# wyf0912/ContextGS

Hardware: AMD Instinct MI355X
Metric: views/sec fwd+bwd @1920×1080, 1M anchors (higher is better)
Workload: dtype f32

## Files before the change

contextgs_amd/csrc/mlp3.hip:

```cpp
#include "cgs_internal.h"
#include "mlp_frag.h"
#include "buf_access.h"

#define M3_IN 54
#define M3_HID 50
#define M3_NTI 4
#define M3_XP 64
#define M3_NT1 4
#define M3_HP 64
#define M3_HCAT 150
#define M3_HLD 150
#define M3_HPITCH 50
#define M3_GLD 192
#define M3_GPITCH 64
#define M3_XLD 54
#ifndef M3_FWD_RT
#define M3_FWD_RT 1
#define M3_FWD_WAVES 16
#ifndef M3_FWD_LDS_STORE
#define M3_FWD_LDS_STORE 1
#endif
#ifndef M3W_ROUTER
#define M3W_ROUTER 1
#endif
#ifndef M3_TAILMAP
#define M3_TAILMAP 1
#endif
#define M3_FWD_PATCH (16 * 70)
#endif
#ifndef M3_BWD_RT
#define M3_BWD_RT 2
#define M3_BWD_WAVES 8
#endif

#ifndef M3_FUSED_WGRAD
#define M3_FUSED_WGRAD 1
#endif
#ifndef M3_PIPE
#define M3_PIPE 0
#endif
#define M3_FENCE()                         \
    do {                                   \
        asm volatile("" ::: "memory");     \
        __builtin_amdgcn_sched_barrier(0); \
    } while (0)

struct M3Head {
    const float *W1, *b1, *W2, *b2;
    float *Y;
    const float *dY;
    float *dZ2;
};

template <int OUT>
struct M3FwdLds {
    static constexpr int NT2 = (OUT + 15) / 16, OP = NT2 * 16;
    static constexpr int S1 = frag_pad4mod8(M3_HP), S2 = frag_pad4mod8(OP);
    static constexpr int FLOATS = M3_XP * S1 + M3_HP * S2 + M3_HP + OP;
};

template <int OUT>
__device__ __forceinline__ void m3_stage_fwd(float *lds, const M3Head &h, int tid, int nthr) {
    using L = M3FwdLds<OUT>;
    float *W1s = lds, *W2s = W1s + M3_XP * L::S1, *b1s = W2s + M3_HP * L::S2, *b2s = b1s + M3_HP;
    frag_stage_transposed<M3_IN, M3_HID, M3_XP, L::S1>(W1s, h.W1, tid, nthr);
    frag_stage_transposed<M3_HID, OUT, M3_HP, L::S2>(W2s, h.W2, tid, nthr);
    for (int i = tid; i < M3_HP; i += nthr) b1s[i] = i < M3_HID ? h.b1[i] : 0.f;
    for (int i = tid; i < L::OP; i += nthr) b2s[i] = i < OUT ? h.b2[i] : 0.f;
}

#define M3_MAX_ROWS (4ll << 20)
struct M3FwdBufs { ClBuf H, Y[3], Xo, X, src, feat, anc; };

template <int OUT, int ACT, int RT, bool TILED, bool TM>
__device__ __forceinline__ void m3_head_fwd(const float *lds, const M3Head &h, int head, const f32x4 (&xb)[RT][M3_NTI],
                                            const bool (&valid)[RT], int64_t row0, int g, int c,
                                            float *__restrict__ Hcat, const M3FwdBufs &B, float *patch) {
    using L = M3FwdLds<OUT>;
    const float *W1s = lds, *W2s = W1s + M3_XP * L::S1, *b1s = W2s + M3_HP * L::S2, *b2s = b1s + M3_HP;
    f32x4 acc1[M3_NT1][RT];
#pragma unroll
    for (int t = 0; t < M3_NT1; ++t)
#pragma unroll
        for (int rt = 0; rt < RT; ++rt) acc1[t][rt] = (f32x4){0.f, 0.f, 0.f, 0.f};
#if M3_PIPE
    float a1[2][4][M3_NT1];
#pragma unroll
    for (int j = 0; j < 4; ++j)
#pragma unroll
        for (int t = 0; t < M3_NT1; ++t) a1[0][j][t] = W1s[(4 * g + j) * L::S1 + 16 * t + c];
    auto krow = [&](int q, int j) { return (TM && q == M3_NTI - 1) ? 16 * q + g + 4 * j : 16 * q + 4 * g + j; };
#pragma unroll
    for (int q = 0; q < M3_NTI; ++q) {
        if (q + 1 < M3_NTI) {
#pragma unroll
            for (int j = 0; j < 4; ++j)
#pragma unroll
                for (int t = 0; t < M3_NT1; ++t)
                    a1[(q + 1) & 1][j][t] = W1s[krow(q + 1, j) * L::S1 + 16 * t + c];
        }
        M3_FENCE();
#pragma unroll
        for (int j = 0; j < 4; ++j) {
            if (16 * q + j >= M3_IN) continue;
            if (TM && q == M3_NTI - 1 && 16 * q + 4 * j >= M3_IN) continue;
#pragma unroll
            for (int t = 0; t < M3_NT1; ++t)
#pragma unroll
                for (int rt = 0; rt < RT; ++rt) acc1[t][rt] = frag_mfma(a1[q & 1][j][t], xb[rt][q][j], acc1[t][rt]);
        }
        M3_FENCE();
    }
#else
#pragma unroll
    for (int q = 0; q < M3_NTI; ++q)
#pragma unroll
        for (int j = 0; j < 4; ++j) {
            if (16 * q + j >= M3_IN) continue;
            if (TM && q == M3_NTI - 1 && 16 * q + 4 * j >= M3_IN) continue;
#pragma unroll
            for (int t = 0; t < M3_NT1; ++t) {
                const float a = W1s[((TM && q == M3_NTI - 1) ? 16 * q + g + 4 * j : 16 * q + 4 * g + j) * L::S1 + 16 * t + c];
#pragma unroll
                for (int rt = 0; rt < RT; ++rt) acc1[t][rt] = frag_mfma(a, xb[rt][q][j], acc1[t][rt]);
            }
        }
#endif
#pragma unroll
    for (int t = 0; t < M3_NT1; ++t)
#pragma unroll
        for (int rt = 0; rt < RT; ++rt) {
            const int64_t row = row0 + rt * 16 + c;
#pragma unroll
            for (int r = 0; r < 4; ++r) acc1[t][rt][r] = fmaxf(acc1[t][rt][r] + b1s[16 * t + 4 * g + r], 0.f);
            if (TILED)
                frag_tstore4<M3_HID>(B.H, (uint32_t)((row0 + rt * 16) >> 4) * (16 * M3_HLD * 4) + (uint32_t)head * (16 * M3_HID * 4), t, g, c,
                                     valid[rt], acc1[t][rt]);
            else
                frag_bstore4<M3_HID>(B.H, (uint32_t)row * (M3_HLD * 4) + (uint32_t)(M3_HPITCH * head) * 4, t, g, valid[rt], acc1[t][rt]);
        }
    f32x4 acc2[L::NT2][RT];
#pragma unroll
    for (int u = 0; u < L::NT2; ++u)
#pragma unroll
        for (int rt = 0; rt < RT; ++rt) acc2[u][rt] = (f32x4){0.f, 0.f, 0.f, 0.f};
#if M3_PIPE
    float a2[2][4][L::NT2];
#pragma unroll
    for (int r = 0; r < 4; ++r)
#pragma unroll
        for (int u = 0; u < L::NT2; ++u) a2[0][r][u] = W2s[(4 * g + r) * L::S2 + 16 * u + c];
#pragma unroll
    for (int t = 0; t < M3_NT1; ++t) {
        if (t + 1 < M3_NT1) {
#pragma unroll
            for (int r = 0; r < 4; ++r) {
                if (16 * (t + 1) + r >= M3_HID) continue;
#pragma unroll
                for (int u = 0; u < L::NT2; ++u) a2[(t + 1) & 1][r][u] = W2s[(16 * (t + 1) + 4 * g + r) * L::S2 + 16 * u + c];
            }
        }
        M3_FENCE();
#pragma unroll
        for (int r = 0; r < 4; ++r) {
            if (16 * t + r >= M3_HID) continue;
#pragma unroll
            for (int u = 0; u < L::NT2; ++u)
#pragma unroll
                for (int rt = 0; rt < RT; ++rt) acc2[u][rt] = frag_mfma(a2[t & 1][r][u], acc1[t][rt][r], acc2[u][rt]);
        }
        M3_FENCE();
    }
#else
#pragma unroll
    for (int t = 0; t < M3_NT1; ++t)
#pragma unroll
        for (int r = 0; r < 4; ++r) {
            if (16 * t + r >= M3_HID) continue;
#pragma unroll
            for (int u = 0; u < L::NT2; ++u) {
                const float a = W2s[(16 * t + 4 * g + r) * L::S2 + 16 * u + c];
#pragma unroll
                for (int rt = 0; rt < RT; ++rt) acc2[u][rt] = frag_mfma(a, acc1[t][rt][r], acc2[u][rt]);
            }
        }
#endif
#if M3_FWD_LDS_STORE
#pragma unroll
    for (int rt = 0; rt < RT; ++rt) {
        f32x4 yv[L::NT2];
#pragma unroll
        for (int u = 0; u < L::NT2; ++u)
#pragma unroll
            for (int r = 0; r < 4; ++r) yv[u][r] = frag_act<ACT>(acc2[u][rt][r] + b2s[16 * u + 4 * g + r]);
        frag_tile_store<OUT, L::NT2>(patch, B.Y[head], (uint32_t)(row0 + rt * 16) * (OUT * 4), yv, g, c, 16 * g + c);
    }
#else
#pragma unroll
    for (int u = 0; u < L::NT2; ++u)
#pragma unroll
        for (int rt = 0; rt < RT; ++rt) {
            const int64_t row = row0 + rt * 16 + c;
            f32x4 y;
#pragma unroll
            for (int r = 0; r < 4; ++r) y[r] = frag_act<ACT>(acc2[u][rt][r] + b2s[16 * u + 4 * g + r]);
            frag_bstore4<OUT>(B.Y[head], (uint32_t)row * (OUT * 4), u, g, valid[rt], y);
        }
#endif
}

struct M3Rows {
    const float *feat_src;
    const int64_t *src_row;
    const float *anchor;
    const float *cam;
    float *X_out;
    float *d_feat_src;
    float *d_anchor;
};

template <bool TM = false>
__device__ __forceinline__ f32x4 m3_load_x_rows_b(const M3FwdBufs &B, float cam0, float cam1, float cam2, int64_t row, int64_t srow,
                                                  int q, int g, bool valid) {
    const uint32_t fo = (uint32_t)srow * (M3_HID * 4);
    if (q < 3) return cl_l128(B.feat, cl_sel(valid, fo + (uint32_t)(16 * q + 4 * g) * 4));
    if (TM) {
        const f32x4 f2 = cl_l64(B.feat, cl_sel(valid && g < 2, fo + 48 * 4));
        const f32x4 a = cl_l96(B.anc, cl_sel(valid, (uint32_t)row * 12));
        const float ux = a[0] - cam0, uy = a[1] - cam1, uz = a[2] - cam2;
        const float dist = sqrtf(ux * ux + uy * uy + uz * uz);
        const float s0 = g == 0 ? f2[0] : (g == 1 ? f2[1] : (g == 2 ? ux / dist : uy / dist));
        const float s1 = g == 0 ? uz / dist : (g == 1 ? dist : 0.f);
        return valid ? (f32x4){s0, s1, 0.f, 0.f} : (f32x4){0.f, 0.f, 0.f, 0.f};
    }
    const f32x4 f2 = cl_l64(B.feat, cl_sel(valid && g == 0, fo + 48 * 4));
    const f32x4 a = cl_l96(B.anc, cl_sel(valid && g < 2, (uint32_t)row * 12));
    const float ux = a[0] - cam0, uy = a[1] - cam1, uz = a[2] - cam2;
    const float dist = sqrtf(ux * ux + uy * uy + uz * uz);
    const f32x4 v0 = (f32x4){f2[0], f2[1], ux / dist, uy / dist}, v1 = (f32x4){uz / dist, dist, 0.f, 0.f};
    const f32x4 z = (f32x4){0.f, 0.f, 0.f, 0.f};
    return !valid ? z : (g == 0 ? v0 : (g == 1 ? v1 : z));
}

template <int O0, int A0, int O1, int A1, int O2, int A2, int RT, int WAVES, bool ROWS, bool TILED = false>
__global__ void __launch_bounds__(WAVES * 64)
    mlp3_fwd_kernel(const float *__restrict__ X, int64_t ldx, M3Head h0, M3Head h1, M3Head h2,
                    float *__restrict__ Hcat, int64_t n, M3Rows R) {
    constexpr int WFL = M3FwdLds<O0>::FLOATS + M3FwdLds<O1>::FLOATS + M3FwdLds<O2>::FLOATS;
    static_assert(WFL % 4 == 0 && O0 <= 70 && O1 <= 70 && O2 <= 70 && M3_IN <= 70, "patch: 16-byte aligned, the widest image fits");
    __shared__ __attribute__((aligned(16))) float lds[WFL + (M3_FWD_LDS_STORE ? WAVES * M3_FWD_PATCH : 0)];
    float *l0 = lds, *l1 = l0 + M3FwdLds<O0>::FLOATS, *l2 = l1 + M3FwdLds<O1>::FLOATS;
    const int tid = threadIdx.x, nthr = WAVES * 64;
    float *patch = lds + WFL + (M3_FWD_LDS_STORE ? (tid >> 6) * M3_FWD_PATCH : 0);
    m3_stage_fwd<O0>(l0, h0, tid, nthr);
    m3_stage_fwd<O1>(l1, h1, tid, nthr);
    m3_stage_fwd<O2>(l2, h2, tid, nthr);
    __syncthreads();
    const int lane = tid & 63, wave = tid >> 6, g = lane >> 4, c = lane & 15;
    const int64_t ntiles = (n + 16 * RT - 1) / (16 * RT);
    f32x4 xb[RT][M3_NTI], xn[RT][M3_NTI];
    bool valid[RT], validn[RT];
    const int64_t tile0 = (int64_t)blockIdx.x * WAVES + wave, tstride = (int64_t)gridDim.x * WAVES;
    M3FwdBufs B;
    {
        const uint64_t nb = (uint64_t)n;
        const uint64_t nbt = (nb + 15) / 16 * 16;
        B.H = cl_buf(Hcat, (TILED ? nbt : nb) * (M3_HLD * 4));
        B.Y[0] = cl_buf(h0.Y, nb * (O0 * 4)); B.Y[1] = cl_buf(h1.Y, nb * (O1 * 4)); B.Y[2] = cl_buf(h2.Y, nb * (O2 * 4));
        B.Xo = cl_buf(ROWS ? R.X_out : nullptr, nb * (M3_XLD * 4));
        B.X = cl_buf(ROWS ? nullptr : X, nb > 0 ? ((nb - 1) * (uint64_t)ldx + M3_IN) * 4 : 0);
        B.src = cl_buf(ROWS ? R.src_row : nullptr, nb * 8);
        B.feat = cl_buf(ROWS ? R.feat_src : nullptr, CL_MAX_BYTES);
        B.anc = cl_buf(ROWS ? R.anchor : nullptr, nb * 12);
    }
    const float cam0 = ROWS ? R.cam[0] : 0.f, cam1 = ROWS ? R.cam[1] : 0.f, cam2 = ROWS ? R.cam[2] : 0.f;
    const uint32_t ldx4 = (uint32_t)ldx * 4;
    int64_t srow_n[RT], srow_nn[RT];
#pragma unroll
    for (int rt = 0; rt < RT; ++rt) {
        const int64_t row = tile0 * 16 * RT + rt * 16 + c, rown = row + tstride * 16 * RT;
        valid[rt] = tile0 < ntiles && row < n;
        const int64_t srow = ROWS ? cl_li64(B.src, cl_sel(valid[rt], (uint32_t)row * 8)) : 0;
        srow_n[rt] = ROWS ? cl_li64(B.src, cl_sel(rown < n, (uint32_t)rown * 8)) : 0;
#pragma unroll
        for (int q = 0; q < M3_NTI; ++q)
            xb[rt][q] = ROWS ? m3_load_x_rows_b<M3_TAILMAP>(B, cam0, cam1, cam2, row, srow, q, g, valid[rt])
                             : frag_bmask4<M3_IN>(frag_bload4<M3_IN>(B.X, (uint32_t)row * ldx4, q, g, valid[rt]), q, g);
    }
    for (int64_t tile = tile0; tile < ntiles; tile += tstride) {
        const int64_t row0 = tile * 16 * RT;
        asm volatile("" ::: "memory");
#pragma unroll
        for (int rt = 0; rt < RT; ++rt) {
            const int64_t row = (tile + tstride) * 16 * RT + rt * 16 + c, rownn = row + tstride * 16 * RT;
            validn[rt] = row < n;
            srow_nn[rt] = ROWS ? cl_li64(B.src, cl_sel(rownn < n, (uint32_t)rownn * 8)) : 0;
#pragma unroll
            for (int q = 0; q < M3_NTI; ++q)
                xn[rt][q] = ROWS ? m3_load_x_rows_b<M3_TAILMAP>(B, cam0, cam1, cam2, row, srow_n[rt], q, g, validn[rt])
                                 : frag_bmask4<M3_IN>(frag_bload4<M3_IN>(B.X, (uint32_t)row * ldx4, q, g, validn[rt]), q, g);
        }
        if (ROWS) {
#pragma unroll
            for (int rt = 0; rt < RT; ++rt)
#if M3_FWD_LDS_STORE
                if (R.X_out) {
                    if (M3_TAILMAP) {
#pragma unroll
                        for (int q = 0; q < M3_NTI - 1; ++q) cl_patch_put4(patch + c * M3_IN + 16 * q + 4 * g, xb[rt][q], 4);
                        patch[c * M3_IN + 48 + g] = xb[rt][M3_NTI - 1][0];
                        if (g < 2) patch[c * M3_IN + 52 + g] = xb[rt][M3_NTI - 1][1];
                        cl_patch_flush<64 * M3_IN>(patch, B.Xo, (uint32_t)(row0 + rt * 16) * (M3_XLD * 4), lane);
                    } else {
                        frag_tile_store<M3_IN, M3_NTI>(patch, B.Xo, (uint32_t)(row0 + rt * 16) * (M3_XLD * 4), xb[rt], g, c, lane);
                    }
                }
#else
#pragma unroll
                for (int q = 0; q < M3_NTI; ++q)
                    frag_bstore4<M3_IN>(B.Xo, (uint32_t)(row0 + rt * 16 + c) * (M3_XLD * 4), q, g, valid[rt], xb[rt][q]);
#endif
        }
        m3_head_fwd<O0, A0, RT, TILED, ROWS && M3_TAILMAP>(l0, h0, 0, xb, valid, row0, g, c, Hcat, B, patch);
        m3_head_fwd<O1, A1, RT, TILED, ROWS && M3_TAILMAP>(l1, h1, 1, xb, valid, row0, g, c, Hcat, B, patch);
        m3_head_fwd<O2, A2, RT, TILED, ROWS && M3_TAILMAP>(l2, h2, 2, xb, valid, row0, g, c, Hcat, B, patch);
#pragma unroll
        for (int rt = 0; rt < RT; ++rt) {
            valid[rt] = validn[rt];
            srow_n[rt] = srow_nn[rt];
#pragma unroll
            for (int q = 0; q < M3_NTI; ++q) xb[rt][q] = xn[rt][q];
        }
    }
}

template <int OUT>
struct M3BwdLds {
    static constexpr int NT2 = (OUT + 15) / 16, OP = NT2 * 16;
    static constexpr int SA = frag_pad4mod8(M3_HP), SB = frag_pad4mod8(M3_XP);
    static constexpr int FLOATS = OP * SA + M3_HP * SB;
};

template <int OUT>
__device__ __forceinline__ void m3_stage_bwd(float *lds, const M3Head &h, int tid, int nthr) {
    using L = M3BwdLds<OUT>;
    float *W2n = lds, *W1n = W2n + L::OP * L::SA;
    frag_stage_loop(h.W2, L::OP * L::SA, tid, nthr,
                    [](int i) { const int o = i / L::SA, hh = i % L::SA; return (o < OUT && hh < M3_HID) ? o * M3_HID + hh : -1; },
                    [&](int i, float v) { W2n[i] = v; });
    frag_stage_loop(h.W1, M3_HP * L::SB, tid, nthr,
                    [](int i) { const int hh = i / L::SB, k = i % L::SB; return (hh < M3_HID && k < M3_IN) ? hh * M3_IN + k : -1; },
                    [&](int i, float v) { W1n[i] = v; });
}

template <int OUT, int ACT, int RT>
__device__ __forceinline__ void m3_head_bwd(const float *lds, const M3Head &h, int head, const bool (&valid)[RT],
                                            int64_t row0, int g, int c, const float *__restrict__ Hcat,
                                            float *__restrict__ dZ1cat, f32x4 (&adx)[M3_NTI][RT]) {
    using L = M3BwdLds<OUT>;
    const float *W2n = lds, *W1n = W2n + L::OP * L::SA;
    f32x4 adh[M3_NT1][RT];
#pragma unroll
    for (int t = 0; t < M3_NT1; ++t)
#pragma unroll
        for (int rt = 0; rt < RT; ++rt) adh[t][rt] = (f32x4){0.f, 0.f, 0.f, 0.f};
    f32x4 b[L::NT2][RT], yv[L::NT2][RT], hv[M3_NT1][RT];
#pragma unroll
    for (int u = 0; u < L::NT2; ++u)
#pragma unroll
        for (int rt = 0; rt < RT; ++rt) {
            const int64_t row = row0 + rt * 16 + c;
            b[u][rt] = frag_load4<OUT>(h.dY + row * OUT, u, g, valid[rt]);
            if (ACT != FRAG_ACT_NONE) yv[u][rt] = frag_load4<OUT>(h.Y + row * OUT, u, g, valid[rt]);
        }
#pragma unroll
    for (int t = 0; t < M3_NT1; ++t)
#pragma unroll
        for (int rt = 0; rt < RT; ++rt)
            hv[t][rt] = frag_load4<M3_HID>(Hcat + (row0 + rt * 16 + c) * M3_HLD + M3_HPITCH * head, t, g, valid[rt]);
    if (ACT != FRAG_ACT_NONE) {
#pragma unroll
        for (int u = 0; u < L::NT2; ++u)
#pragma unroll
            for (int rt = 0; rt < RT; ++rt) {
#pragma unroll
                for (int r = 0; r < 4; ++r) b[u][rt][r] *= frag_act_grad<ACT>(yv[u][rt][r]);
                frag_store4<OUT>(h.dZ2 + (row0 + rt * 16 + c) * OUT, u, g, valid[rt], b[u][rt]);
            }
    }
#pragma unroll
    for (int u = 0; u < L::NT2; ++u)
#pragma unroll
        for (int j = 0; j < 4; ++j) {
            if (16 * u + j >= OUT) continue;
#pragma unroll
            for (int t = 0; t < M3_NT1; ++t) {
                const float a = W2n[(16 * u + 4 * g + j) * L::SA + 16 * t + c];
#pragma unroll
                for (int rt = 0; rt < RT; ++rt) adh[t][rt] = frag_mfma(a, b[u][rt][j], adh[t][rt]);
            }
        }
#pragma unroll
    for (int t = 0; t < M3_NT1; ++t)
#pragma unroll
        for (int rt = 0; rt < RT; ++rt) {
            const int64_t at = (row0 + rt * 16 + c) * M3_GLD + M3_GPITCH * head;
#pragma unroll
            for (int r = 0; r < 4; ++r) adh[t][rt][r] = hv[t][rt][r] > 0.f ? adh[t][rt][r] : 0.f;
// ... 55 lines not shown
                    dst[49] = adx[3][rt][1];
                    const float dvx = adx[3][rt][2], dvy = adx[3][rt][3], dvz = z52, dd = z53;
                    const float ux = R.anchor[3 * row] - R.cam[0], uy = R.anchor[3 * row + 1] - R.cam[1],
                                uz = R.anchor[3 * row + 2] - R.cam[2];
                    const float dist = sqrtf(ux * ux + uy * uy + uz * uz), inv = 1.f / dist;
                    const float vx = ux * inv, vy = uy * inv, vz = uz * inv;
                    const float dot = vx * dvx + vy * dvy + vz * dvz;
                    R.d_anchor[3 * row] = (dvx - vx * dot) * inv + vx * dd;
                    R.d_anchor[3 * row + 1] = (dvy - vy * dot) * inv + vy * dd;
                    R.d_anchor[3 * row + 2] = (dvz - vz * dot) * inv + vz * dd;
                }
            }
        } else if (dX) {
#pragma unroll
            for (int v = 0; v < M3_NTI; ++v)
#pragma unroll
                for (int rt = 0; rt < RT; ++rt)
                    frag_store4<M3_IN>(dX + (row0 + rt * 16 + c) * lddx, v, g, valid[rt], adx[v][rt]);
        }
    }
}


#define M3W_LD 20
#ifndef M3W_XPREFETCH
#define M3W_XPREFETCH 1
#endif
#define M3W_PATCH (16 * M3W_LD)
#ifndef M3W_PREFETCH_AT
#define M3W_PREFETCH_AT 2
#endif
#ifndef M3W_EARLY
#define M3W_EARLY 0
#endif
#define M3W_NPATCH 13
#define M3W_WAVES 4
#define M3W_E (M3_GLD * (M3_IN + 1) + (10 + 30 + 70) * (M3_HID + 1))

__device__ __forceinline__ f32x4 m3w_f2n(float *patch, f32x4 v, int g, int c) {
    *(f32x4 *)(patch + c * M3W_LD + 4 * g) = v;
    f32x4 o;
#pragma unroll
    for (int r = 0; r < 4; ++r) o[r] = patch[(4 * g + r) * M3W_LD + c];
    return o;
}

struct M3wBufs { ClBuf dY[3], Y[3], H, X; };
template <int OUT, int ACT>
struct M3wOps {
    static constexpr int NT2 = (OUT + 15) / 16;
    f32x4 dy[NT2], y[ACT != FRAG_ACT_NONE ? NT2 : 1], h[M3_NT1];
    template <bool TILED = false>
    __device__ __forceinline__ void load(const M3wBufs &B, int head, int64_t row, int g, bool valid) {
        const uint32_t ro = (uint32_t)row * (OUT * 4), rh = (uint32_t)row * (M3_HLD * 4) + (uint32_t)(M3_HPITCH * head) * 4;
        const uint32_t th = (uint32_t)(row >> 4) * (16 * M3_HLD * 4) + (uint32_t)head * (16 * M3_HID * 4);
#pragma unroll
        for (int u = 0; u < NT2; ++u) {
            dy[u] = frag_bload4<OUT>(B.dY[head], ro, u, g, valid);
            if (ACT != FRAG_ACT_NONE) y[u] = frag_bload4<OUT>(B.Y[head], ro, u, g, valid);
        }
#pragma unroll
        for (int t = 0; t < M3_NT1; ++t)
            h[t] = TILED ? frag_tload4<M3_HID>(B.H, th, t, g, (int)(row & 15), valid) : frag_bload4<M3_HID>(B.H, rh, t, g, valid);
    }
    __device__ __forceinline__ void mask(int g) {
#pragma unroll
        for (int u = 0; u < NT2; ++u) {
            dy[u] = frag_bmask4<OUT>(dy[u], u, g);
            if (ACT != FRAG_ACT_NONE) y[u] = frag_bmask4<OUT>(y[u], u, g);
        }
#pragma unroll
        for (int t = 0; t < M3_NT1; ++t) h[t] = frag_bmask4<M3_HID>(h[t], t, g);
    }
};

__device__ __forceinline__ void m3w_put(float *patch, f32x4 v, int g, int c) { *(f32x4 *)(patch + c * M3W_LD + 4 * g) = v; }
__device__ __forceinline__ f32x4 m3w_get(const float *patch, int g, int c) {
    f32x4 o;
#pragma unroll
    for (int r = 0; r < 4; ++r) o[r] = patch[(4 * g + r) * M3W_LD + c];
    return o;
}

template <int OUT, int ACT, class Prefetch>
__device__ __forceinline__ void m3w_head(const float *lds, float *patches, M3wOps<OUT, ACT> &op, f32x4 ones, int g, int c,
                                         const f32x4 (&xn)[M3_NTI], f32x4 (&adx)[M3_NTI],
                                         f32x4 (&aw2)[(OUT + 15) / 16][M3_NT1], f32x4 (&aw1)[M3_NT1][M3_NTI], Prefetch prefetch) {
    using L = M3BwdLds<OUT>;
    const float *W2n = lds, *W1n = W2n + L::OP * L::SA;
    op.mask(g);
    f32x4 b[L::NT2];
#pragma unroll
    for (int u = 0; u < L::NT2; ++u) {
        b[u] = op.dy[u];
        if (ACT != FRAG_ACT_NONE) {
#pragma unroll
            for (int r = 0; r < 4; ++r) b[u][r] *= frag_act_grad<ACT>(op.y[u][r]);
        }
    }
#pragma unroll
    for (int t = 0; t < M3_NT1; ++t) m3w_put(patches + t * M3W_PATCH, op.h[t], g, c);
#pragma unroll
    for (int u = 0; u < L::NT2; ++u) m3w_put(patches + (4 + u) * M3W_PATCH, b[u], g, c);
    if (M3W_PREFETCH_AT == 0) prefetch();
    auto ldw2 = [&](int u, int j) {
        f32x4 w;
#pragma unroll
        for (int t = 0; t < M3_NT1; ++t) w[t] = W2n[(16 * u + 4 * g + j) * L::SA + 16 * t + c];
        return w;
    };
    auto ldw1 = [&](int t, int r) {
        f32x4 w;
#pragma unroll
        for (int v = 0; v < M3_NTI; ++v) w[v] = W1n[(16 * t + 4 * g + r) * L::SB + 16 * v + c];
        return w;
    };
    f32x4 adh[M3_NT1], hn[M3_NT1], zc;
#pragma unroll
    for (int t = 0; t < M3_NT1; ++t) adh[t] = (f32x4){0.f, 0.f, 0.f, 0.f};
    {
        f32x4 wc = ldw2(0, 0);
        if (M3W_EARLY) {
#pragma unroll
            for (int t = 0; t < M3_NT1; ++t) hn[t] = m3w_get(patches + t * M3W_PATCH, g, c);
            zc = m3w_get(patches + 4 * M3W_PATCH, g, c);
        }
#pragma unroll
        for (int u = 0; u < L::NT2; ++u)
#pragma unroll
            for (int j = 0; j < 4; ++j) {
                if (16 * u + j >= OUT) continue;
                const int un = j == 3 ? u + 1 : u, jn = j == 3 ? 0 : j + 1;
                f32x4 wn = wc;
                if (un < L::NT2 && 16 * un + jn < OUT) wn = ldw2(un, jn);
                M3_FENCE();
#pragma unroll
                for (int t = 0; t < M3_NT1; ++t) adh[t] = frag_mfma(wc[t], b[u][j], adh[t]);
                M3_FENCE();
                wc = wn;
            }
    }
    if (M3W_PREFETCH_AT == 1) prefetch();
#pragma unroll
    for (int t = 0; t < M3_NT1; ++t) {
#pragma unroll
        for (int r = 0; r < 4; ++r) adh[t][r] = op.h[t][r] > 0.f ? adh[t][r] : 0.f;
        m3w_put(patches + (9 + t) * M3W_PATCH, adh[t], g, c);
    }
    if (!M3W_EARLY) {
#pragma unroll
        for (int t = 0; t < M3_NT1; ++t) hn[t] = m3w_get(patches + t * M3W_PATCH, g, c);
        zc = m3w_get(patches + 4 * M3W_PATCH, g, c);
    }
    if (c == M3_HID - 48) hn[3] = ones;
    f32x4 wx, dc;
    if (M3W_EARLY) {
        wx = ldw1(0, 0);
        dc = m3w_get(patches + 9 * M3W_PATCH, g, c);
    }
#pragma unroll
    for (int u = 0; u < L::NT2; ++u) {
        f32x4 zn = zc;
        if (u + 1 < L::NT2) zn = m3w_get(patches + (4 + u + 1) * M3W_PATCH, g, c);
        M3_FENCE();
#if M3W_ROUTER
#pragma unroll
        for (int r = 0; r < 4; ++r)
#pragma unroll
            for (int t = 0; t < M3_NT1; ++t) aw2[u][t] = frag_mfma(zc[r], hn[t][r], aw2[u][t]);
#else
#pragma unroll
        for (int t = 0; t < M3_NT1; ++t)
#pragma unroll
            for (int r = 0; r < 4; ++r) aw2[u][t] = frag_mfma(zc[r], hn[t][r], aw2[u][t]);
#endif
        M3_FENCE();
        zc = zn;
    }
    if (M3W_PREFETCH_AT == 2) prefetch();
    if (!M3W_EARLY) wx = ldw1(0, 0);
#pragma unroll
    for (int t = 0; t < M3_NT1; ++t)
#pragma unroll
        for (int r = 0; r < 4; ++r) {
            if (16 * t + r >= M3_HID) continue;
            const int tn = r == 3 ? t + 1 : t, rn = r == 3 ? 0 : r + 1;
            f32x4 wn = wx;
            if (tn < M3_NT1 && 16 * tn + rn < M3_HID) wn = ldw1(tn, rn);
            M3_FENCE();
#pragma unroll
            for (int v = 0; v < M3_NTI; ++v) adx[v] = frag_mfma(wx[v], adh[t][r], adx[v]);
            M3_FENCE();
            wx = wn;
        }
    if (!M3W_EARLY) dc = m3w_get(patches + 9 * M3W_PATCH, g, c);
#pragma unroll
    for (int t = 0; t < M3_NT1; ++t) {
        f32x4 dn = dc;
        if (t + 1 < M3_NT1) dn = m3w_get(patches + (9 + t + 1) * M3W_PATCH, g, c);
        M3_FENCE();
#if M3W_ROUTER
#pragma unroll
        for (int r = 0; r < 4; ++r)
#pragma unroll
            for (int v = 0; v < M3_NTI; ++v) aw1[t][v] = frag_mfma(dc[r], xn[v][r], aw1[t][v]);
#else
#pragma unroll
        for (int v = 0; v < M3_NTI; ++v)
#pragma unroll
            for (int r = 0; r < 4; ++r) aw1[t][v] = frag_mfma(dc[r], xn[v][r], aw1[t][v]);
#endif
        M3_FENCE();
        dc = dn;
    }
}

template <bool ROWS, bool TL = false>
__global__ void __launch_bounds__(M3W_WAVES * 64) __attribute__((amdgpu_waves_per_eu(1, 1)))
    mlp3_bwd_wg_kernel(M3Head h0, M3Head h1, M3Head h2, const float *__restrict__ X, int64_t ldx,
                       const float *__restrict__ Hcat, float *__restrict__ dX, int64_t lddx, int64_t n, M3Rows R,
                       float *__restrict__ partial) {
    constexpr int WF = M3BwdLds<10>::FLOATS + M3BwdLds<30>::FLOATS + M3BwdLds<70>::FLOATS;
    constexpr int PF = M3W_WAVES * M3W_NPATCH * M3W_PATCH;
    static_assert(WF + PF >= M3W_E, "the LDS image of the weight gradients reuses the weight region");
    __shared__ __attribute__((aligned(16))) float lds[WF + PF];
    float *l0 = lds, *l1 = l0 + M3BwdLds<10>::FLOATS, *l2 = l1 + M3BwdLds<30>::FLOATS;
    const int tid = threadIdx.x, nthr = M3W_WAVES * 64;
    m3_stage_bwd<10>(l0, h0, tid, nthr);
    m3_stage_bwd<30>(l1, h1, tid, nthr);
    m3_stage_bwd<70>(l2, h2, tid, nthr);
    __syncthreads();
    const int lane = tid & 63, wave = tid >> 6, g = lane >> 4, c = lane & 15;
    float *patches = lds + WF + wave * M3W_NPATCH * M3W_PATCH;
    const int64_t ntiles = (n + 15) / 16;
    f32x4 a2_0[1][M3_NT1], a2_1[2][M3_NT1], a2_2[5][M3_NT1], a1_0[M3_NT1][M3_NTI], a1_1[M3_NT1][M3_NTI], a1_2[M3_NT1][M3_NTI];
    const f32x4 zero = (f32x4){0.f, 0.f, 0.f, 0.f};
#pragma unroll
    for (int t = 0; t < M3_NT1; ++t) {
        a2_0[0][t] = zero;
#pragma unroll
        for (int u = 0; u < 2; ++u) a2_1[u][t] = zero;
#pragma unroll
        for (int u = 0; u < 5; ++u) a2_2[u][t] = zero;
#pragma unroll
        for (int v = 0; v < M3_NTI; ++v) { a1_0[t][v] = zero; a1_1[t][v] = zero; a1_2[t][v] = zero; }
    }
    const int64_t tstride = (int64_t)gridDim.x * M3W_WAVES;
    int64_t tile = (int64_t)blockIdx.x * M3W_WAVES + wave;
    const uint64_t nb = (uint64_t)n;
    M3wBufs B;
    B.dY[0] = cl_buf(h0.dY, nb * 40); B.dY[1] = cl_buf(h1.dY, nb * 120); B.dY[2] = cl_buf(h2.dY, nb * 280);
    B.Y[0] = cl_buf(h0.Y, nb * 40); B.Y[1] = cl_buf(h1.Y, nb * 120); B.Y[2] = cl_buf(h2.Y, nb * 280);
    static_assert(ROWS || !TL, "the tiled hand-over belongs to the ROWS pair");
    B.H = cl_buf(Hcat, (TL ? (nb + 15) / 16 * 16 : nb) * (M3_HLD * 4));
    B.X = cl_buf(X, nb > 0 ? ((nb - 1) * (uint64_t)ldx + M3_IN) * 4 : 0);
    const ClBuf bSrc = cl_buf(ROWS ? R.src_row : nullptr, nb * 8), bAnc = cl_buf(ROWS ? R.anchor : nullptr, nb * 12);
    const float cam0 = ROWS ? R.cam[0] : 0.f, cam1 = ROWS ? R.cam[1] : 0.f, cam2 = ROWS ? R.cam[2] : 0.f;
    const uint32_t ldx4 = (uint32_t)ldx * 4;
    const bool regather = ROWS && X == nullptr;
    M3FwdBufs FB;
    FB.feat = cl_buf(regather ? R.feat_src : nullptr, CL_MAX_BYTES);
    FB.anc = bAnc;
    auto load_x = [&](f32x4 (&x)[M3_NTI], int64_t row, int64_t srow, bool v) {
#pragma unroll
        for (int q = 0; q < M3_NTI; ++q)
            x[q] = regather ? m3_load_x_rows_b(FB, cam0, cam1, cam2, row, srow, q, g, v)
                            : frag_bload4<M3_IN>(B.X, (uint32_t)row * ldx4, q, g, v);
    };
    M3wOps<10, 1> op0;
    M3wOps<30, 2> op1;
    M3wOps<70, 0> op2;
    f32x4 xf[M3_NTI];
    int64_t srow_next = 0;
    {
        const int64_t row = tile * 16 + c;
        const bool v0 = tile < ntiles && row < n;
        op0.template load<TL>(B, 0, row, g, v0);
        const int64_t s0 = regather ? cl_li64(bSrc, cl_sel(v0, (uint32_t)row * 8)) : 0;
        load_x(xf, row, s0, v0);
    }
    for (; tile < ntiles; tile += tstride) {
        const int64_t row0 = tile * 16;
        asm volatile("" ::: "memory");
        const bool valid = row0 + c < n;
        const int64_t rown = row0 + tstride * 16 + c;
        const bool validn = rown < n;
        f32x4 ones, xn[M3_NTI];
#pragma unroll
        for (int r = 0; r < 4; ++r) ones[r] = row0 + 4 * g + r < n ? 1.f : 0.f;
        const int64_t srow_pre = ROWS ? cl_li64(bSrc, cl_sel(valid, (uint32_t)(row0 + c) * 8)) : 0;
#if !M3W_XPREFETCH
        load_x(xf, row0 + c, srow_pre, valid);
#endif
        if (regather) srow_next = cl_li64(bSrc, cl_sel(validn, (uint32_t)rown * 8));
        const f32x4 anc_pre = ROWS ? cl_l96(bAnc, cl_sel(valid && g == 0, (uint32_t)(row0 + c) * 12)) : zero;
#pragma unroll
        for (int q = 0; q < M3_NTI; ++q) m3w_put(patches + q * M3W_PATCH, frag_bmask4<M3_IN>(xf[q], q, g), g, c);
#pragma unroll
        for (int q = 0; q < M3_NTI; ++q) xn[q] = m3w_get(patches + q * M3W_PATCH, g, c);
        if (c == M3_IN - 48) xn[3] = ones;
        f32x4 adx[M3_NTI];
#pragma unroll
        for (int v = 0; v < M3_NTI; ++v) adx[v] = zero;
        m3w_head<10, 1>(l0, patches, op0, ones, g, c, xn, adx, a2_0, a1_0, [&]() { op1.template load<TL>(B, 1, row0 + c, g, valid); });
        m3w_head<30, 2>(l1, patches, op1, ones, g, c, xn, adx, a2_1, a1_1, [&]() { op2.template load<TL>(B, 2, row0 + c, g, valid); });
        m3w_head<70, 0>(l2, patches, op2, ones, g, c, xn, adx, a2_2, a1_2, [&]() {
            op0.template load<TL>(B, 0, rown, g, validn);
#if M3W_XPREFETCH
            load_x(xf, rown, srow_next, validn);
#endif
        });
        if (ROWS) {
            const int64_t row = row0 + c;
            const int64_t srow = valid ? srow_pre : 0;
            float *dst = R.d_feat_src + srow * M3_HID;
#pragma unroll
            for (int v = 0; v < 3; ++v)
                if (valid) *(f32x4_a4 *)(dst + 16 * v + 4 * g) = adx[v];
            const float z52 = __shfl(adx[3][0], 16 + c, 64), z53 = __shfl(adx[3][1], 16 + c, 64);
            if (g == 0 && valid) {
                dst[48] = adx[3][0];
                dst[49] = adx[3][1];
                const float dvx = adx[3][2], dvy = adx[3][3], dvz = z52, dd = z53;
                const float ux = anc_pre[0] - cam0, uy = anc_pre[1] - cam1, uz = anc_pre[2] - cam2;
                const float dist = sqrtf(ux * ux + uy * uy + uz * uz), inv = 1.f / dist;
                const float vx = ux * inv, vy = uy * inv, vz = uz * inv;
                const float dot = vx * dvx + vy * dvy + vz * dvz;
                R.d_anchor[3 * row] = (dvx - vx * dot) * inv + vx * dd;
                R.d_anchor[3 * row + 1] = (dvy - vy * dot) * inv + vy * dd;
                R.d_anchor[3 * row + 2] = (dvz - vz * dot) * inv + vz * dd;
            }
        } else if (dX) {
#pragma unroll
            for (int v = 0; v < M3_NTI; ++v) frag_store4<M3_IN>(dX + (row0 + c) * lddx, v, g, valid, adx[v]);
        }
    }
    __syncthreads();
    for (int i = tid; i < M3W_E; i += nthr) lds[i] = 0.f;
    __syncthreads();
    float *img1 = lds, *imgb1 = img1 + M3_GLD * M3_IN;
    for (int w = 0; w < M3W_WAVES; ++w) {
        if (wave == w) {
#pragma unroll
            for (int hd = 0; hd < 3; ++hd) {
                const f32x4 (&a1)[M3_NT1][M3_NTI] = hd == 0 ? a1_0 : (hd == 1 ? a1_1 : a1_2);
#pragma unroll
                for (int t = 0; t < M3_NT1; ++t)
#pragma unroll
                    for (int v = 0; v < M3_NTI; ++v)
#pragma unroll
                        for (int r = 0; r < 4; ++r) {
                            const int m = M3_GPITCH * hd + 16 * t + 4 * g + r, k = 16 * v + c;
                            if (k < M3_IN) img1[m * M3_IN + k] += a1[t][v][r];
                            else if (k == M3_IN) imgb1[m] += a1[t][v][r];
                        }
            }
            float *img2 = imgb1 + M3_GLD;
#define M3W_IMG2(ACC, NT2_, OUT_)                                                          \
            {                                                                               \
                _Pragma("unroll") for (int u = 0; u < NT2_; ++u)                            \
                _Pragma("unroll") for (int t = 0; t < M3_NT1; ++t)                          \
                _Pragma("unroll") for (int r = 0; r < 4; ++r) {                             \
                    const int o = 16 * u + 4 * g + r, hh = 16 * t + c;                      \
                    if (o < OUT_) {                                                         \
                        if (hh < M3_HID) img2[o * M3_HID + hh] += ACC[u][t][r];             \
                        else if (hh == M3_HID) img2[OUT_ * M3_HID + o] += ACC[u][t][r];     \
                    }                                                                       \
                }                                                                           \
                img2 += OUT_ * (M3_HID + 1);                                                \
            }
            M3W_IMG2(a2_0, 1, 10)
            M3W_IMG2(a2_1, 2, 30)
            M3W_IMG2(a2_2, 5, 70)
#undef M3W_IMG2
        }
        __syncthreads();
    }
    float *dstp = partial + (int64_t)blockIdx.x * M3W_E;
    for (int i = tid; i < M3W_E; i += nthr) dstp[i] = lds[i];
}


static int m3_cus() {
    static int cus = 0;
    if (!cus) {
        int dev = 0;
        hipDeviceProp_t p;
        if (hipGetDevice(&dev) == hipSuccess && hipGetDeviceProperties(&p, dev) == hipSuccess) cus = p.multiProcessorCount;
        if (cus <= 0) cus = 256;
    }
    return cus;
}

extern "C" int cgs_anchor_mlp3_layout(int *out4) {
    if (!out4) { cgs_set_error("cgs_anchor_mlp3_layout: NULL"); return CGS_ERR_ARG; }
    out4[0] = M3_HLD; out4[1] = M3_XLD; out4[2] = M3_GLD; out4[3] = M3_GPITCH;
    return CGS_OK;
}

extern "C" int cgs_anchor_mlp3_forward(const float *X, int64_t ldx, const float *const *W1, const float *const *b1,
                                       const float *const *W2, const float *const *b2, float *Y_op, float *Y_color,
                                       float *Y_cov, float *Hcat, int64_t n, void *stream) {
    if (n < 0) { cgs_set_error("anchor_mlp3_forward: n < 0"); return CGS_ERR_ARG; }
    if (n == 0) return CGS_OK;
    if (!X || !W1 || !b1 || !W2 || !b2 || !Y_op || !Y_color || !Y_cov) { cgs_set_error("anchor_mlp3_forward: NULL"); return CGS_ERR_ARG; }
    constexpr int RT = M3_FWD_RT, WAVES = M3_FWD_WAVES;
    M3Head h[3];
    float *ys[3] = {Y_op, Y_color, Y_cov};
    for (int i = 0; i < 3; ++i) h[i] = M3Head{W1[i], b1[i], W2[i], b2[i], ys[i], nullptr, nullptr};
    if (ldx < M3_IN || ldx > 4096) { cgs_set_error("anchor_mlp3_forward: ldx out of range"); return CGS_ERR_ARG; }
    CgsProfScope prof(CGS_PROF_MLP_FWD, (hipStream_t)stream);
    const int64_t step = ldx <= 256 ? M3_MAX_ROWS : M3_MAX_ROWS / 16;
    for (int64_t r0 = 0; r0 < n; r0 += step) {
        const int64_t m = n - r0 < step ? n - r0 : step;
        for (int i = 0; i < 3; ++i) h[i].Y = ys[i] + r0 * (i == 0 ? 10 : (i == 1 ? 30 : 70));
        const int64_t tiles = (m + 16 * RT - 1) / (16 * RT);
        const int64_t want = (tiles + WAVES - 1) / WAVES;
        const int grid = (int)(want < m3_cus() ? want : m3_cus());
        hipLaunchKernelGGL((mlp3_fwd_kernel<10, 1, 30, 2, 70, 0, RT, WAVES, false>), dim3(grid), dim3(WAVES * 64), 0, (hipStream_t)stream,
                           X + r0 * ldx, ldx, h[0], h[1], h[2], Hcat ? Hcat + r0 * M3_HLD : nullptr, m, M3Rows{});
    }
    CGS_CHECK_HIP(hipGetLastError());
    return CGS_OK;
}

extern "C" int cgs_anchor_mlp3_forward_rows_t(const float *feat_src, const int64_t *src_row, const float *anchor_vis,
                                              const float *cam3, float *X_out, const float *const *W1,
                                              const float *const *b1, const float *const *W2, const float *const *b2,
                                              float *Y_op, float *Y_color, float *Y_cov, float *Hcat, int64_t n, int tiled,
                                              void *stream);
extern "C" int cgs_anchor_mlp3_forward_rows(const float *feat_src, const int64_t *src_row, const float *anchor_vis,
                                            const float *cam3, float *X_out, const float *const *W1,
                                            const float *const *b1, const float *const *W2, const float *const *b2,
                                            float *Y_op, float *Y_color, float *Y_cov, float *Hcat, int64_t n, void *stream) {
    return cgs_anchor_mlp3_forward_rows_t(feat_src, src_row, anchor_vis, cam3, X_out, W1, b1, W2, b2, Y_op, Y_color, Y_cov, Hcat, n, 0,
                                          stream);
}
extern "C" int cgs_anchor_mlp3_forward_rows_t(const float *feat_src, const int64_t *src_row, const float *anchor_vis,
// ... 185 lines not shown
```

Baseline: 162.1.

## Pack hidden-unit tails of three MLP heads into one shared MFMA tile

The hidden layer has 50 units, so the fourth 16-wide MFMA tile per head held only 2 useful units. The change runs 48 units per head in three tiles and packs the leftover units of all three heads into a single shared tail tile, with matching W2 row remapping. In the backward weight gradient the tail dH is gathered into a shared patch so one MFMA set accumulates W1 gradients for all three tails. This removes roughly two padded MFMA tiles per row-tile in forward and backward. The cost is extra LDS staging, index remapping and cross-head coupling through the shared patch, with correctness risk in the packed row mapping.

```diff
diff --git a/contextgs_amd/csrc/mlp3.hip b/contextgs_amd/csrc/mlp3.hip
--- a/contextgs_amd/csrc/mlp3.hip
+++ b/contextgs_amd/csrc/mlp3.hip
@@ -33,6 +33,20 @@
 #define M3_BWD_WAVES 8
 #endif
 
+#ifndef M3_PACK
+#define M3_PACK 1
+#endif
+#define M3_NT1F (M3_PACK ? 3 : M3_NT1)
+#define M3_TS 20
+__device__ __forceinline__ int m3_w2row(int hh, int h) { return (M3_PACK && hh >= 48) ? 48 + 4 * h + (hh - 48) : hh; }
+__device__ __forceinline__ int m3_w2unit(int row, int h) {
+    if (!M3_PACK || row < 48) return row < M3_HID ? row : -1;
+    const int gg = (row - 48) >> 2, j = (row - 48) & 3;
+    return (gg == h && j < M3_HID - 48) ? 48 + j : -1;
+}
+__device__ __forceinline__ int m3_tail_head(int p) { return p >> 2 < 3 ? p >> 2 : 2; }
+__device__ __forceinline__ int m3_tail_unit(int p) { return (p >> 2 < 3 && (p & 3) < M3_HID - 48) ? 48 + (p & 3) : -1; }
+
 #ifndef M3_FUSED_WGRAD
 #define M3_FUSED_WGRAD 1
 #endif
@@ -54,41 +68,65 @@
 
 template <int OUT>
 struct M3FwdLds {
-    static constexpr int NT2 = (OUT + 15) / 16, OP = NT2 * 16;
-    static constexpr int S1 = frag_pad4mod8(M3_HP), S2 = frag_pad4mod8(OP);
-    static constexpr int FLOATS = M3_XP * S1 + M3_HP * S2 + M3_HP + OP;
+    static constexpr int NT2 = (OUT + 15) / 16, OP = NT2 * 16, HP1 = 16 * M3_NT1F;
+    static constexpr int S1 = frag_pad4mod8(HP1), S2 = frag_pad4mod8(OP);
+    static constexpr int FLOATS = M3_XP * S1 + M3_HP * S2 + HP1 + OP;
 };
+struct M3FwdTail {
+    static constexpr int FLOATS = M3_PACK ? M3_XP * M3_TS + 16 : 0;
+};
 
 template <int OUT>
-__device__ __forceinline__ void m3_stage_fwd(float *lds, const M3Head &h, int tid, int nthr) {
+__device__ __forceinline__ void m3_stage_fwd(float *lds, const M3Head &h, int head, int tid, int nthr) {
     using L = M3FwdLds<OUT>;
-    float *W1s = lds, *W2s = W1s + M3_XP * L::S1, *b1s = W2s + M3_HP * L::S2, *b2s = b1s + M3_HP;
-    frag_stage_transposed<M3_IN, M3_HID, M3_XP, L::S1>(W1s, h.W1, tid, nthr);
-    frag_stage_transposed<M3_HID, OUT, M3_HP, L::S2>(W2s, h.W2, tid, nthr);
-    for (int i = tid; i < M3_HP; i += nthr) b1s[i] = i < M3_HID ? h.b1[i] : 0.f;
+    float *W1s = lds, *W2s = W1s + M3_XP * L::S1, *b1s = W2s + M3_HP * L::S2, *b2s = b1s + L::HP1;
+    constexpr int HID1 = M3_PACK ? 48 : M3_HID;
+    frag_stage_transposed<M3_IN, HID1, M3_XP, L::S1>(W1s, h.W1, tid, nthr);
+    for (int i = tid; i < M3_HP * L::S2; i += nthr) {
+        const int r = i / L::S2, o = i % L::S2;
+        if (o >= OUT || m3_w2unit(r, head) < 0) W2s[i] = 0.f;
+    }
+    frag_stage_loop(h.W2, OUT * M3_HID, tid, nthr, [](int i) { return i; },
+                    [&](int i, float v) { const int o = i / M3_HID, hh = i % M3_HID; W2s[m3_w2row(hh, head) * L::S2 + o] = v; });
+    for (int i = tid; i < L::HP1; i += nthr) b1s[i] = i < HID1 ? h.b1[i] : 0.f;
     for (int i = tid; i < L::OP; i += nthr) b2s[i] = i < OUT ? h.b2[i] : 0.f;
+}
+
+__device__ __forceinline__ void m3_stage_fwd_tail(float *lds, const M3Head &h0, const M3Head &h1, const M3Head &h2, int tid, int nthr) {
+    float *W1t = lds, *b1t = W1t + M3_XP * M3_TS;
+    for (int i = tid; i < M3_XP * M3_TS; i += nthr) {
+        const int k = i / M3_TS, p = i % M3_TS;
+        if (k >= M3_IN || p >= 16 || m3_tail_unit(p) < 0) W1t[i] = 0.f;
+    }
+    constexpr int NU = M3_HID - 48;
+    for (int i = tid; i < 3 * NU * M3_IN; i += nthr) {
+        const int hd = i / (NU * M3_IN), j = (i / M3_IN) % NU, k = i % M3_IN;
+        const float *W1 = hd == 0 ? h0.W1 : (hd == 1 ? h1.W1 : h2.W1);
+        W1t[k * M3_TS + 4 * hd + j] = W1[(48 + j) * M3_IN + k];
+    }
+    for (int p = tid; p < 16; p += nthr) {
+        const int hd = m3_tail_head(p), u = m3_tail_unit(p);
+        const float *b1 = hd == 0 ? h0.b1 : (hd == 1 ? h1.b1 : h2.b1);
+        b1t[p] = u < 0 ? 0.f : b1[u];
+    }
 }
 
 #define M3_MAX_ROWS (4ll << 20)
 struct M3FwdBufs { ClBuf H, Y[3], Xo, X, src, feat, anc; };
 
-template <int OUT, int ACT, int RT, bool TILED, bool TM>
-__device__ __forceinline__ void m3_head_fwd(const float *lds, const M3Head &h, int head, const f32x4 (&xb)[RT][M3_NTI],
-                                            const bool (&valid)[RT], int64_t row0, int g, int c,
-                                            float *__restrict__ Hcat, const M3FwdBufs &B, float *patch) {
-    using L = M3FwdLds<OUT>;
-    const float *W1s = lds, *W2s = W1s + M3_XP * L::S1, *b1s = W2s + M3_HP * L::S2, *b2s = b1s + M3_HP;
-    f32x4 acc1[M3_NT1][RT];
-#pragma unroll
-    for (int t = 0; t < M3_NT1; ++t)
+template <int NT, int S, int RT, bool TM>
+__device__ __forceinline__ void m3_layer1(const float *W1s, const float *b1s, const f32x4 (&xb)[RT][M3_NTI], int g, int c,
+                                          f32x4 (&acc1)[NT][RT]) {
+#pragma unroll
+    for (int t = 0; t < NT; ++t)
 #pragma unroll
         for (int rt = 0; rt < RT; ++rt) acc1[t][rt] = (f32x4){0.f, 0.f, 0.f, 0.f};
 #if M3_PIPE
-    float a1[2][4][M3_NT1];
+    float a1[2][4][NT];
 #pragma unroll
     for (int j = 0; j < 4; ++j)
 #pragma unroll
-        for (int t = 0; t < M3_NT1; ++t) a1[0][j][t] = W1s[(4 * g + j) * L::S1 + 16 * t + c];
+        for (int t = 0; t < NT; ++t) a1[0][j][t] = W1s[(4 * g + j) * S + 16 * t + c];
     auto krow = [&](int q, int j) { return (TM && q == M3_NTI - 1) ? 16 * q + g + 4 * j : 16 * q + 4 * g + j; };
 #pragma unroll
     for (int q = 0; q < M3_NTI; ++q) {
@@ -96,8 +134,8 @@
 #pragma unroll
             for (int j = 0; j < 4; ++j)
 #pragma unroll
-                for (int t = 0; t < M3_NT1; ++t)
-                    a1[(q + 1) & 1][j][t] = W1s[krow(q + 1, j) * L::S1 + 16 * t + c];
+                for (int t = 0; t < NT; ++t)
+                    a1[(q + 1) & 1][j][t] = W1s[krow(q + 1, j) * S + 16 * t + c];
         }
         M3_FENCE();
 #pragma unroll
@@ -105,7 +143,7 @@
             if (16 * q + j >= M3_IN) continue;
             if (TM && q == M3_NTI - 1 && 16 * q + 4 * j >= M3_IN) continue;
 #pragma unroll
-            for (int t = 0; t < M3_NT1; ++t)
+            for (int t = 0; t < NT; ++t)
 #pragma unroll
                 for (int rt = 0; rt < RT; ++rt) acc1[t][rt] = frag_mfma(a1[q & 1][j][t], xb[rt][q][j], acc1[t][rt]);
         }
@@ -119,26 +157,41 @@
             if (16 * q + j >= M3_IN) continue;
             if (TM && q == M3_NTI - 1 && 16 * q + 4 * j >= M3_IN) continue;
 #pragma unroll
-            for (int t = 0; t < M3_NT1; ++t) {
-                const float a = W1s[((TM && q == M3_NTI - 1) ? 16 * q + g + 4 * j : 16 * q + 4 * g + j) * L::S1 + 16 * t + c];
+            for (int t = 0; t < NT; ++t) {
+                const float a = W1s[((TM && q == M3_NTI - 1) ? 16 * q + g + 4 * j : 16 * q + 4 * g + j) * S + 16 * t + c];
 #pragma unroll
                 for (int rt = 0; rt < RT; ++rt) acc1[t][rt] = frag_mfma(a, xb[rt][q][j], acc1[t][rt]);
             }
         }
 #endif
 #pragma unroll
-    for (int t = 0; t < M3_NT1; ++t)
+    for (int t = 0; t < NT; ++t)
+#pragma unroll
+        for (int rt = 0; rt < RT; ++rt)
+#pragma unroll
+            for (int r = 0; r < 4; ++r) acc1[t][rt][r] = fmaxf(acc1[t][rt][r] + b1s[16 * t + 4 * g + r], 0.f);
+}
+
+template <int OUT, int ACT, int RT, bool TILED, bool TM>
+__device__ __forceinline__ void m3_head_fwd(const float *lds, const M3Head &h, int head, const f32x4 (&xb)[RT][M3_NTI],
+                                            const f32x4 (&acct)[RT], const bool (&valid)[RT], int64_t row0, int g, int c,
+                                            float *__restrict__ Hcat, const M3FwdBufs &B, float *patch) {
+    using L = M3FwdLds<OUT>;
+    const float *W1s = lds, *W2s = W1s + M3_XP * L::S1, *b1s = W2s + M3_HP * L::S2, *b2s = b1s + L::HP1;
+    f32x4 acc1[M3_NT1F][RT];
+    m3_layer1<M3_NT1F, L::S1, RT, TM>(W1s, b1s, xb, g, c, acc1);
+#pragma unroll
+    for (int t = 0; t < M3_NT1F; ++t)
 #pragma unroll
         for (int rt = 0; rt < RT; ++rt) {
             const int64_t row = row0 + rt * 16 + c;
-#pragma unroll
-            for (int r = 0; r < 4; ++r) acc1[t][rt][r] = fmaxf(acc1[t][rt][r] + b1s[16 * t + 4 * g + r], 0.f);
             if (TILED)
                 frag_tstore4<M3_HID>(B.H, (uint32_t)((row0 + rt * 16) >> 4) * (16 * M3_HLD * 4) + (uint32_t)head * (16 * M3_HID * 4), t, g, c,
                                      valid[rt], acc1[t][rt]);
             else
                 frag_bstore4<M3_HID>(B.H, (uint32_t)row * (M3_HLD * 4) + (uint32_t)(M3_HPITCH * head) * 4, t, g, valid[rt], acc1[t][rt]);
         }
+    auto hid = [&](int t, int rt, int r) { return (M3_PACK && t >= M3_NT1F) ? acct[rt][r] : acc1[t < M3_NT1F ? t : 0][rt][r]; };
     f32x4 acc2[L::NT2][RT];
 #pragma unroll
     for (int u = 0; u < L::NT2; ++u)
@@ -167,7 +220,7 @@
 #pragma unroll
             for (int u = 0; u < L::NT2; ++u)
 #pragma unroll
-                for (int rt = 0; rt < RT; ++rt) acc2[u][rt] = frag_mfma(a2[t & 1][r][u], acc1[t][rt][r], acc2[u][rt]);
+                for (int rt = 0; rt < RT; ++rt) acc2[u][rt] = frag_mfma(a2[t & 1][r][u], hid(t, rt, r), acc2[u][rt]);
         }
         M3_FENCE();
     }
@@ -181,7 +234,7 @@
             for (int u = 0; u < L::NT2; ++u) {
                 const float a = W2s[(16 * t + 4 * g + r) * L::S2 + 16 * u + c];
 #pragma unroll
-                for (int rt = 0; rt < RT; ++rt) acc2[u][rt] = frag_mfma(a, acc1[t][rt][r], acc2[u][rt]);
+                for (int rt = 0; rt < RT; ++rt) acc2[u][rt] = frag_mfma(a, hid(t, rt, r), acc2[u][rt]);
             }
         }
 #endif
@@ -246,15 +299,16 @@
 __global__ void __launch_bounds__(WAVES * 64)
     mlp3_fwd_kernel(const float *__restrict__ X, int64_t ldx, M3Head h0, M3Head h1, M3Head h2,
                     float *__restrict__ Hcat, int64_t n, M3Rows R) {
-    constexpr int WFL = M3FwdLds<O0>::FLOATS + M3FwdLds<O1>::FLOATS + M3FwdLds<O2>::FLOATS;
+    constexpr int WFL = M3FwdLds<O0>::FLOATS + M3FwdLds<O1>::FLOATS + M3FwdLds<O2>::FLOATS + M3FwdTail::FLOATS;
     static_assert(WFL % 4 == 0 && O0 <= 70 && O1 <= 70 && O2 <= 70 && M3_IN <= 70, "patch: 16-byte aligned, the widest image fits");
     __shared__ __attribute__((aligned(16))) float lds[WFL + (M3_FWD_LDS_STORE ? WAVES * M3_FWD_PATCH : 0)];
-    float *l0 = lds, *l1 = l0 + M3FwdLds<O0>::FLOATS, *l2 = l1 + M3FwdLds<O1>::FLOATS;
+    float *l0 = lds, *l1 = l0 + M3FwdLds<O0>::FLOATS, *l2 = l1 + M3FwdLds<O1>::FLOATS, *lt = l2 + M3FwdLds<O2>::FLOATS;
     const int tid = threadIdx.x, nthr = WAVES * 64;
     float *patch = lds + WFL + (M3_FWD_LDS_STORE ? (tid >> 6) * M3_FWD_PATCH : 0);
-    m3_stage_fwd<O0>(l0, h0, tid, nthr);
-    m3_stage_fwd<O1>(l1, h1, tid, nthr);
-    m3_stage_fwd<O2>(l2, h2, tid, nthr);
+    m3_stage_fwd<O0>(l0, h0, 0, tid, nthr);
+    m3_stage_fwd<O1>(l1, h1, 1, tid, nthr);
+    m3_stage_fwd<O2>(l2, h2, 2, tid, nthr);
+    if (M3_PACK) m3_stage_fwd_tail(lt, h0, h1, h2, tid, nthr);
     __syncthreads();
     const int lane = tid & 63, wave = tid >> 6, g = lane >> 4, c = lane & 15;
     const int64_t ntiles = (n + 16 * RT - 1) / (16 * RT);
@@ -321,9 +375,23 @@
                     frag_bstore4<M3_IN>(B.Xo, (uint32_t)(row0 + rt * 16 + c) * (M3_XLD * 4), q, g, valid[rt], xb[rt][q]);
 #endif
         }
-        m3_head_fwd<O0, A0, RT, TILED, ROWS && M3_TAILMAP>(l0, h0, 0, xb, valid, row0, g, c, Hcat, B, patch);
-        m3_head_fwd<O1, A1, RT, TILED, ROWS && M3_TAILMAP>(l1, h1, 1, xb, valid, row0, g, c, Hcat, B, patch);
-        m3_head_fwd<O2, A2, RT, TILED, ROWS && M3_TAILMAP>(l2, h2, 2, xb, valid, row0, g, c, Hcat, B, patch);
+        f32x4 acct[1][RT];
+        if (M3_PACK) {
+            m3_layer1<1, M3_TS, RT, ROWS && M3_TAILMAP>(lt, lt + M3_XP * M3_TS, xb, g, c, acct);
+            const int hd = m3_tail_head(4 * g);
+#pragma unroll
+            for (int rt = 0; rt < RT; ++rt) {
+                if (TILED)
+                    frag_tstore4<M3_HID>(B.H, (uint32_t)((row0 + rt * 16) >> 4) * (16 * M3_HLD * 4) + (uint32_t)hd * (16 * M3_HID * 4), 3, 0, c,
+                                         valid[rt] && g < 3, acct[0][rt]);
+                else
+                    frag_bstore4<M3_HID>(B.H, (uint32_t)(row0 + rt * 16 + c) * (M3_HLD * 4) + (uint32_t)(M3_HPITCH * hd) * 4, 3, 0,
+                                         valid[rt] && g < 3, acct[0][rt]);
+            }
+        }
+        m3_head_fwd<O0, A0, RT, TILED, ROWS && M3_TAILMAP>(l0, h0, 0, xb, acct[0], valid, row0, g, c, Hcat, B, patch);
+        m3_head_fwd<O1, A1, RT, TILED, ROWS && M3_TAILMAP>(l1, h1, 1, xb, acct[0], valid, row0, g, c, Hcat, B, patch);
+        m3_head_fwd<O2, A2, RT, TILED, ROWS && M3_TAILMAP>(l2, h2, 2, xb, acct[0], valid, row0, g, c, Hcat, B, patch);
 #pragma unroll
         for (int rt = 0; rt < RT; ++rt) {
             valid[rt] = validn[rt];
@@ -545,10 +613,11 @@
     return o;
 }
 
-template <int OUT, int ACT, class Prefetch>
+template <int OUT, int ACT, int HEAD, class Prefetch>
 __device__ __forceinline__ void m3w_head(const float *lds, float *patches, M3wOps<OUT, ACT> &op, f32x4 ones, int g, int c,
                                          const f32x4 (&xn)[M3_NTI], f32x4 (&adx)[M3_NTI],
-                                         f32x4 (&aw2)[(OUT + 15) / 16][M3_NT1], f32x4 (&aw1)[M3_NT1][M3_NTI], Prefetch prefetch) {
+                                         f32x4 (&aw2)[(OUT + 15) / 16][M3_NT1], f32x4 (&aw1)[M3_NT1F][M3_NTI],
+                                         f32x4 (&aw1t)[M3_NTI], Prefetch prefetch) {
     using L = M3BwdLds<OUT>;
     const float *W2n = lds, *W1n = W2n + L::OP * L::SA;
     op.mask(g);
@@ -608,7 +677,11 @@
     for (int t = 0; t < M3_NT1; ++t) {
 #pragma unroll
         for (int r = 0; r < 4; ++r) adh[t][r] = op.h[t][r] > 0.f ? adh[t][r] : 0.f;
-        m3w_put(patches + (9 + t) * M3W_PATCH, adh[t], g, c);
+        if (M3_PACK && t >= M3_NT1F) {
+            if (g == 0) *(f32x4 *)(patches + 12 * M3W_PATCH + c * M3W_LD + 4 * HEAD) = adh[t];
+        } else {
+            m3w_put(patches + (9 + t) * M3W_PATCH, adh[t], g, c);
+        }
     }
     if (!M3W_EARLY) {
 #pragma unroll
@@ -656,22 +729,24 @@
             M3_FENCE();
             wx = wn;
         }
+    constexpr int NTW = (M3_PACK && HEAD < 2) ? M3_NT1F : M3_NT1;
     if (!M3W_EARLY) dc = m3w_get(patches + 9 * M3W_PATCH, g, c);
 #pragma unroll
-    for (int t = 0; t < M3_NT1; ++t) {
+    for (int t = 0; t < NTW; ++t) {
         f32x4 dn = dc;
-        if (t + 1 < M3_NT1) dn = m3w_get(patches + (9 + t + 1) * M3W_PATCH, g, c);
+        if (t + 1 < NTW) dn = m3w_get(patches + (9 + t + 1) * M3W_PATCH, g, c);
+        f32x4 (&aw)[M3_NTI] = (M3_PACK && t >= M3_NT1F) ? aw1t : aw1[t < M3_NT1F ? t : 0];
         M3_FENCE();
 #if M3W_ROUTER
 #pragma unroll
         for (int r = 0; r < 4; ++r)
 #pragma unroll
-            for (int v = 0; v < M3_NTI; ++v) aw1[t][v] = frag_mfma(dc[r], xn[v][r], aw1[t][v]);
+            for (int v = 0; v < M3_NTI; ++v) aw[v] = frag_mfma(dc[r], xn[v][r], aw[v]);
 #else
 #pragma unroll
         for (int v = 0; v < M3_NTI; ++v)
 #pragma unroll
-            for (int r = 0; r < 4; ++r) aw1[t][v] = frag_mfma(dc[r], xn[v][r], aw1[t][v]);
+            for (int r = 0; r < 4; ++r) aw[v] = frag_mfma(dc[r], xn[v][r], aw[v]);
 #endif
         M3_FENCE();
         dc = dn;
@@ -696,7 +771,8 @@
     const int lane = tid & 63, wave = tid >> 6, g = lane >> 4, c = lane & 15;
     float *patches = lds + WF + wave * M3W_NPATCH * M3W_PATCH;
     const int64_t ntiles = (n + 15) / 16;
-    f32x4 a2_0[1][M3_NT1], a2_1[2][M3_NT1], a2_2[5][M3_NT1], a1_0[M3_NT1][M3_NTI], a1_1[M3_NT1][M3_NTI], a1_2[M3_NT1][M3_NTI];
+    f32x4 a2_0[1][M3_NT1], a2_1[2][M3_NT1], a2_2[5][M3_NT1], a1_0[M3_NT1F][M3_NTI], a1_1[M3_NT1F][M3_NTI], a1_2[M3_NT1F][M3_NTI];
+    f32x4 a1_t[M3_NTI];
     const f32x4 zero = (f32x4){0.f, 0.f, 0.f, 0.f};
 #pragma unroll
     for (int t = 0; t < M3_NT1; ++t) {
@@ -706,8 +782,13 @@
 #pragma unroll
         for (int u = 0; u < 5; ++u) a2_2[u][t] = zero;
 #pragma unroll
-        for (int v = 0; v < M3_NTI; ++v) { a1_0[t][v] = zero; a1_1[t][v] = zero; a1_2[t][v] = zero; }
-    }
+        for (int v = 0; v < M3_NTI; ++v) {
+            a1_0[t < M3_NT1F ? t : 0][v] = zero; a1_1[t < M3_NT1F ? t : 0][v] = zero; a1_2[t < M3_NT1F ? t : 0][v] = zero;
+        }
+    }
+#pragma unroll
+    for (int v = 0; v < M3_NTI; ++v) a1_t[v] = zero;
+    if (M3_PACK && g == 3) m3w_put(patches + 12 * M3W_PATCH, zero, g, c);
     const int64_t tstride = (int64_t)gridDim.x * M3W_WAVES;
     int64_t tile = (int64_t)blockIdx.x * M3W_WAVES + wave;
     const uint64_t nb = (uint64_t)n;
@@ -765,9 +846,9 @@
         f32x4 adx[M3_NTI];
 #pragma unroll
         for (int v = 0; v < M3_NTI; ++v) adx[v] = zero;
-        m3w_head<10, 1>(l0, patches, op0, ones, g, c, xn, adx, a2_0, a1_0, [&]() { op1.template load<TL>(B, 1, row0 + c, g, valid); });
-        m3w_head<30, 2>(l1, patches, op1, ones, g, c, xn, adx, a2_1, a1_1, [&]() { op2.template load<TL>(B, 2, row0 + c, g, valid); });
-        m3w_head<70, 0>(l2, patches, op2, ones, g, c, xn, adx, a2_2, a1_2, [&]() {
+        m3w_head<10, 1, 0>(l0, patches, op0, ones, g, c, xn, adx, a2_0, a1_0, a1_t, [&]() { op1.template load<TL>(B, 1, row0 + c, g, valid); });
+        m3w_head<30, 2, 1>(l1, patches, op1, ones, g, c, xn, adx, a2_1, a1_1, a1_t, [&]() { op2.template load<TL>(B, 2, row0 + c, g, valid); });
+        m3w_head<70, 0, 2>(l2, patches, op2, ones, g, c, xn, adx, a2_2, a1_2, a1_t, [&]() {
             op0.template load<TL>(B, 0, rown, g, validn);
 #if M3W_XPREFETCH
             load_x(xf, rown, srow_next, validn);
@@ -806,9 +887,9 @@
         if (wave == w) {
 #pragma unroll
             for (int hd = 0; hd < 3; ++hd) {
-                const f32x4 (&a1)[M3_NT1][M3_NTI] = hd == 0 ? a1_0 : (hd == 1 ? a1_1 : a1_2);
-#pragma unroll
-                for (int t = 0; t < M3_NT1; ++t)
+                const f32x4 (&a1)[M3_NT1F][M3_NTI] = hd == 0 ? a1_0 : (hd == 1 ? a1_1 : a1_2);
+#pragma unroll
+                for (int t = 0; t < M3_NT1F; ++t)
 #pragma unroll
                     for (int v = 0; v < M3_NTI; ++v)
 #pragma unroll
@@ -817,6 +898,17 @@
                             if (k < M3_IN) img1[m * M3_IN + k] += a1[t][v][r];
                             else if (k == M3_IN) imgb1[m] += a1[t][v][r];
                         }
+            }
+            if (M3_PACK) {
+#pragma unroll
+                for (int v = 0; v < M3_NTI; ++v)
+#pragma unroll
+                    for (int r = 0; r < 4; ++r) {
+                        const int u = m3_tail_unit(4 * g + r), m = M3_GPITCH * m3_tail_head(4 * g + r) + u, k = 16 * v + c;
+                        if (u < 0) continue;
+                        if (k < M3_IN) img1[m * M3_IN + k] += a1_t[v][r];
+                        else if (k == M3_IN) imgb1[m] += a1_t[v][r];
+                    }
             }
             float *img2 = imgb1 + M3_GLD;
 #define M3W_IMG2(ACC, NT2_, OUT_)                                                          \
```

New measurement: 164.1 (median of 6 runs). 1.2% higher.
